# chao1224/GeoSSL

Hardware: AMD Instinct MI355X
Metric: molecules/s/GPU SchNet+DDM fwd+bwd (QM9-sized, bs=1024); % HBM roofline (higher is better)
Workload: dtype f32

## Files before the change

### geossl_amd/csrc/aggregate_reg.h

```cpp
#pragma once
#include "common.h"

namespace geossl {

typedef float f32x2 __attribute__((ext_vector_type(2)));

template <int NMAX, int RING_ = 0>
__device__ __forceinline__ void aggregate_reg_body(const float* __restrict__ x, const float* __restrict__ Wf,
                                                   const uint8_t* __restrict__ pair_flag, int a0, int n, int base,
                                                   int lane, int f, int F, int swap, float* __restrict__ out) {
#pragma clang fp contract(off)
  typedef f32x2 V;
#ifndef AGG_RING_SMALL
#define AGG_RING_SMALL 16
#endif
  constexpr int RING = RING_ > 0 ? RING_ : (NMAX > 26 ? 24 : (NMAX > 20 ? 20 : (NMAX > 18 ? 12 : AGG_RING_SMALL)));
  constexpr int NPOS = NMAX * (NMAX - 1) / 2;
  const float* __restrict__ wbase = Wf + (size_t)base * F;
  const bool has_cols = f >= 0;
  f = has_cols ? f : 0;
  if (n < 2) {
    if (n == 1 && has_cols) *reinterpret_cast<V*>(out + (size_t)a0 * F + f) = V(0.0f);
    return;
  }
  V xr[NMAX], acc[NMAX], ring[RING];
#pragma unroll
  for (int i = 0; i < NMAX; ++i) {
    xr[i] = *reinterpret_cast<const V*>(x + (size_t)(a0 + min(i, n - 1)) * F + f);
    acc[i] = V(0.0f);
  }
  const int nu = __builtin_amdgcn_readfirstlane(n);
  int rs_req = 0;
  auto load_row = [&](int a, int b) {
    asm volatile("" : "+s"(rs_req));
    const int slot = b < nu ? rs_req + (b - a - 1) : 0;
    const float* rowp = wbase + (size_t)slot * F;
    return __builtin_nontemporal_load(reinterpret_cast<const V*>(rowp + f));
  };
  auto next_pos = [&](int& a, int& b) {
    if (++b == NMAX) {
      rs_req += nu - a - 1;
      ++a;
      b = a + 1;
    }
  };
  unsigned flr[NMAX - 1];
#pragma unroll
  for (int a = 0; a < NMAX - 1; ++a) {
    const bool mine = lane > a && lane < n;
    flr[a] = pair_flag[base + (mine ? a * n - a * (a + 1) / 2 + lane - a - 1 : 0)];
  }
  int q = 0, ap = 0, bp = 1;
#pragma unroll
  for (int k = 0; k < RING && k < NPOS; ++k) {
    ring[k] = load_row(ap, bp);
    next_pos(ap, bp);
  }
#pragma unroll
  for (int a = 0; a < NMAX - 1; ++a) {
    const bool mine = lane > a && lane < n;
    unsigned fl = flr[a];
    asm volatile("" : "+v"(fl));
    fl = mine ? fl : 0u;
    if (swap) fl = ((fl & 1u) << 1) | ((fl >> 1) & 1u);
    const unsigned long long m0 = __builtin_amdgcn_ballot_w64((fl & 1u) != 0u);
    const unsigned long long m1 = __builtin_amdgcn_ballot_w64((fl & 2u) != 0u);
    V acc_a = acc[a];
    const V xa = xr[a];
#pragma unroll
    for (int b = a + 1; b < NMAX; ++b, ++q) {
      const V w = ring[q % RING];
      if (q + RING < NPOS) {
        ring[q % RING] = load_row(ap, bp);
        next_pos(ap, bp);
      }
      const V t0 = xr[b] * w;
      const V s0 = acc_a + t0;
      acc_a = ((m0 >> b) & 1ull) ? s0 : acc_a;
      const V t1 = xa * w;
      const V s1 = acc[b] + t1;
      acc[b] = ((m1 >> b) & 1ull) ? s1 : acc[b];
      asm volatile("" : "+v"(acc_a.x), "+v"(acc_a.y), "+v"(acc[b].x), "+v"(acc[b].y) : : "memory");
      __builtin_amdgcn_sched_barrier(0);
    }
    acc[a] = acc_a;
  }
#pragma unroll
  for (int i = 0; i < NMAX; ++i)
    if (i < n && has_cols) *reinterpret_cast<V*>(out + (size_t)(a0 + i) * F + f) = acc[i];
}

template <int NW = 4>
__device__ __forceinline__ void aggregate_block_body(const float* __restrict__ x, const float* __restrict__ Wf,
                                                     const uint8_t* __restrict__ pair_flag, int a0, int n, int base,
                                                     int swap, float* __restrict__ out, uint8_t* smem) {
#pragma clang fp contract(off)
  typedef f32x2 V;
  constexpr int F = 128, NP = 32;
  float* xs = reinterpret_cast<float*>(smem);
  uint8_t* fls = smem + 33 * F * sizeof(float);
  const int tid = threadIdx.x, lane = tid & 63;
  const int wave = __builtin_amdgcn_readfirstlane(tid >> 6);
  const int nu = __builtin_amdgcn_readfirstlane(n), np = nu * (nu - 1) / 2;
  for (int i = tid; i < nu * (F / 4); i += 64 * NW) {
    const int row = i >> 5, q = i & 31;
    *reinterpret_cast<f32x4*>(xs + row * F + 4 * q) = *reinterpret_cast<const f32x4*>(x + (size_t)(a0 + row) * F + 4 * q);
  }
  for (int p = tid; p < np; p += 64 * NW) {
    unsigned fl = pair_flag[base + p];
    if (swap) fl = ((fl & 1u) << 1) | ((fl >> 1) & 1u);
    fls[p] = (uint8_t)fl;
  }
  __syncthreads();
  if (nu < 2) {
    if (nu == 1 && wave == 0) *reinterpret_cast<V*>(out + (size_t)a0 * F + 2 * lane) = V(0.0f);
    return;
  }
  const float* __restrict__ wcol = Wf + (size_t)base * F + 2 * lane;
  const float* xl = xs + 2 * lane;
  int slot_l = 0, b_l = 0;
  unsigned long long mask = 0ull;
  auto describe = [&](int a) {
    const int u = lane < nu - 1 ? lane : 0;
    const int b = u + (u >= a ? 1 : 0);
    const int i = min(a, b), j = max(a, b);
    slot_l = nu > 1 ? i * nu - i * (i + 1) / 2 + (j - i - 1) : 0;
    b_l = nu > 1 ? b : 0;
    const unsigned fl = nu > 1 ? (unsigned)fls[slot_l] : 0u;
    const bool sends = lane < nu - 1 && ((a < b ? (fl & 1u) : (fl & 2u)) != 0u);
    mask = __builtin_amdgcn_ballot_w64(sends);
  };
  auto request = [&](V (&w)[NP]) {
#pragma unroll
    for (int u = 0; u < NP; ++u) {
      const int s = __builtin_amdgcn_readlane(slot_l, u);
      w[u] = __builtin_nontemporal_load(reinterpret_cast<const V*>(wcol + (size_t)s * F));
    }
  };
  auto reduce = [&](const V (&w)[NP], int a, unsigned long long m, int bl) {
    V acc = V(0.0f);
#pragma unroll
    for (int u = 0; u < NP; ++u) {
      const int b = __builtin_amdgcn_readlane(bl, u);
      const V xb = *reinterpret_cast<const V*>(xl + b * F);
      const V t = xb * w[u];
      const V s = acc + t;
      acc = ((m >> u) & 1ull) ? s : acc;
    }
    *reinterpret_cast<V*>(out + (size_t)(a0 + a) * F + 2 * lane) = acc;
  };
  V w0[NP], w1[NP];
  int a = wave;
  if (a < nu) {
    describe(a);
    request(w0);
  }
  while (a < nu) {
    const unsigned long long m0 = mask;
    const int bl0 = b_l;
    const int an = a + NW;
    if (an < nu) {
      describe(an);
      request(w1);
    }
    reduce(w0, a, m0, bl0);
    if (an >= nu) break;
    const unsigned long long m1 = mask;
    const int bl1 = b_l;
    const int an2 = an + NW;
    if (an2 < nu) {
      describe(an2);
      request(w0);
    }
    reduce(w1, an, m1, bl1);
    a = an2;
  }
}

__device__ __forceinline__ void aggregate_targets(const float* __restrict__ x, const float* __restrict__ Wf,
                                                  const uint8_t* __restrict__ pair_flag, int a0, int n, int base,
                                                  int lane, int f, int F, int swap, float* __restrict__ out, int t0,
                                                  int t1) {
#pragma clang fp contract(off)
  typedef f32x2 V;
  constexpr int NP = 32;
  const bool has_cols = f >= 0;
  f = has_cols ? f : 0;
  const int nu = __builtin_amdgcn_readfirstlane(n);
  if (nu < 2) {
    if (nu == 1 && t0 == 0 && t1 > 0 && has_cols) *reinterpret_cast<V*>(out + (size_t)a0 * F + f) = V(0.0f);
    return;
  }
  const float* __restrict__ wcol = Wf + (size_t)base * F + f;
  const float* __restrict__ xcol = x + (size_t)a0 * F + f;
  const uint8_t* __restrict__ flg = pair_flag + base;
  for (int a = t0; a < t1; ++a) {
    V acc = V(0.0f);
    for (int c0 = 0; c0 < nu - 1; c0 += NP) {
      const int u = min(c0 + (lane & (NP - 1)), nu - 2);
      const int b = u + (u >= a ? 1 : 0);
      const int i = min(a, b), j = max(a, b);
      const int slot = i * nu - i * (i + 1) / 2 + (j - i - 1);
      unsigned fl = flg[slot];
      if (swap) fl = ((fl & 1u) << 1) | ((fl >> 1) & 1u);
      const bool sends = lane < NP && c0 + lane < nu - 1 && ((a < b ? (fl & 1u) : (fl & 2u)) != 0u);
      const unsigned long long m = __builtin_amdgcn_ballot_w64(sends);
      V w[NP], xb[NP];
#pragma unroll
      for (int k = 0; k < NP; ++k) {
        const int sk = __builtin_amdgcn_readlane(slot, k), bk = __builtin_amdgcn_readlane(b, k);
        w[k] = *reinterpret_cast<const V*>(wcol + (size_t)sk * F);
        xb[k] = *reinterpret_cast<const V*>(xcol + (size_t)bk * F);
      }
      __builtin_amdgcn_sched_barrier(0);
#pragma unroll
      for (int k = 0; k < NP; ++k) {
        const V t = xb[k] * w[k];
        const V s2 = acc + t;
        acc = ((m >> k) & 1ull) ? s2 : acc;
      }
    }
    if (has_cols) *reinterpret_cast<V*>(out + (size_t)(a0 + a) * F + f) = acc;
  }
}

template <int NMAX, int K, int P>
__device__ __forceinline__ void aggregate_reg_part(const float* __restrict__ x, const float* __restrict__ Wf,
                                                   const uint8_t* __restrict__ pair_flag, int a0, int n, int base,
                                                   int lane, int f, int F, int swap, float* __restrict__ out) {
#pragma clang fp contract(off)
  typedef f32x2 V;
  constexpr int G0 = (P * NMAX) / K, G1 = ((P + 1) * NMAX) / K, NG = G1 - G0;
  constexpr int AEND = G1 < NMAX - 1 ? G1 : NMAX - 1;
  constexpr int RING = 40;
#define AGG_BS(a) ((a) < G0 ? G0 : (a) + 1)
#define AGG_BE(a) ((a) < G0 ? G1 : NMAX)
  constexpr int NPOS = G0 * NG + (AEND - G0) * NMAX - ((AEND * (AEND + 1)) / 2 - (G0 * (G0 + 1)) / 2);
  const bool has_cols = f >= 0;
  f = has_cols ? f : 0;
  const float* __restrict__ wbase = Wf + (size_t)base * F;
  V xr[NMAX], acc[NG], ring[RING];
#pragma unroll
// ... 96 lines not shown
```

### geossl_amd/csrc/chain.hip

```cpp
#include "common.h"
#include "geossl_hip.h"
#include "split.h"
#ifdef LOOP_TIMING
__device__ long long loop_dbg[2 * 1024];
__device__ int loop_dbg_n;
#define LOOP_MARK(tag)                                                                                     \
  do {                                                                                                     \
    if (blockIdx.x == 5 && threadIdx.x == 64) {                                                            \
      const int k_ = loop_dbg_n;                                                                           \
      if (k_ < 1024) {                                                                                     \
        loop_dbg[2 * k_] = (tag);                                                                          \
        loop_dbg[2 * k_ + 1] = (long long)__builtin_amdgcn_s_memrealtime();                                \
        loop_dbg_n = k_ + 1;                                                                               \
      }                                                                                                    \
    }                                                                                                      \
  } while (0)
#else
#define LOOP_MARK(tag) do {} while (0)
#endif
#include "aggregate_reg.h"

#include <cstdlib>

using namespace geossl;
// ... 342 lines not shown
#pragma unroll
      for (int s = 0; s < NS; ++s) {
        const GeosslChainStage st = ch.st[s];
        const uint32_t ro = rowc * (uint32_t)st.ld * 4u + 16u * kh;
#pragma unroll
        for (int mb = 0; mb < NMB; ++mb, ++cc) {
          f32x4 tp[4], rs[4];
          if (st.tprev != nullptr) {
            const char* tb = reinterpret_cast<const char*>(st.tprev) + 128 * mb;
#pragma unroll
            for (int q = 0; q < 4; ++q) tp[q] = *reinterpret_cast<const f32x4*>(tb + 32 * q + ro);
          }
          if (st.res != nullptr) {
            const char* rbp = reinterpret_cast<const char*>(st.res) + 128 * mb;
#pragma unroll
            for (int q = 0; q < 4; ++q) rs[q] = *reinterpret_cast<const f32x4*>(rbp + 32 * q + ro);
          }
          f32x16 acc;
#pragma unroll
          for (int q = 0; q < 4; ++q) {
            const f32x4 b = *reinterpret_cast<const f32x4*>(bias_s + s * F + 32 * mb + 8 * q + 4 * kh);
            acc[4 * q] = b.x; acc[4 * q + 1] = b.y; acc[4 * q + 2] = b.z; acc[4 * q + 3] = b.w;
          }
          {
            const u32x4* Ws = ring + (size_t)(cc % NSLOT) * CHUNK + lane;
            Frag3 af, an;
            af.h = Ws[0]; af.m = Ws[64]; af.l = Ws[128];
#pragma unroll
            for (int ks = 0; ks < KS; ++ks) {
              if (ks + 1 < KS) {
                const u32x4* src = Ws + (size_t)((ks + 1) * 3) * 64;
                an.h = src[0]; an.m = src[64]; an.l = src[128];
              }
              __builtin_amdgcn_sched_barrier(0);
              mma6(acc, af, xf[ks]);
              __builtin_amdgcn_sched_barrier(0);
              if (ks + 1 < KS) af = an;
            }
          }
          float v[16];
          epilogue(st, mb, acc, tp, rs, v);
          if (s + 1 < NS) {
            const float lo[8] = {v[0], v[1], v[2], v[3], v[4], v[5], v[6], v[7]};
            const float hi[8] = {v[8], v[9], v[10], v[11], v[12], v[13], v[14], v[15]};
            yf[2 * mb] = split8(lo);
            yf[2 * mb + 1] = split8(hi);
          }
          __syncthreads();
          store_v(st, mb, ro, live, v);
          if (cc + NSLOT < total) issue(cc + NSLOT);
        }
        if (s + 1 < NS) {
#pragma unroll
          for (int ks = 0; ks < KS; ++ks) xf[ks] = yf[ks];
        }
      }
    } else {
      const int m = wave - 4;
      const int rb = base + 4 * B + (int)blockIdx.x;
      const bool active = m < NMB && rb < nrb;
      const int row = 32 * rb + j;
      const bool live = active && row < R;
      const uint32_t rowc = (uint32_t)min(row, R - 1);
      if (active) {
        const char* xb = reinterpret_cast<const char*>(X) + 128 * m;
        const uint32_t xo = rowc * (uint32_t)ldx * 4u + 16u * kh;
        const f32x4 r0 = *reinterpret_cast<const f32x4*>(xb + xo), r1 = *reinterpret_cast<const f32x4*>(xb + 32 + xo);
        const f32x4 r2 = *reinterpret_cast<const f32x4*>(xb + 64 + xo), r3 = *reinterpret_cast<const f32x4*>(xb + 96 + xo);
        const float lo[8] = {r0.x, r0.y, r0.z, r0.w, r1.x, r1.y, r1.z, r1.w};
        const float hi[8] = {r2.x, r2.y, r2.z, r2.w, r3.x, r3.y, r3.z, r3.w};
        const Frag3 f0 = split8(lo), f1 = split8(hi);
        u32x4* xd = xchg + (size_t)CHUNK + (size_t)(2 * m * 3) * 64 + lane;
        xd[0] = f0.h; xd[64] = f0.m; xd[128] = f0.l;
        xd[192] = f1.h; xd[256] = f1.m; xd[320] = f1.l;
      }
      __syncthreads();
#pragma unroll
      for (int s = 0; s < NS; ++s) {
        const GeosslChainStage st = ch.st[s];
#pragma unroll
        for (int mbc = 0; mbc < NMB; ++mbc, ++cc) {
          float v[16];
          uint32_t ro = 0;
          if (active && mbc == 0) {
            const char* img = reinterpret_cast<const char*>(st.image) + (size_t)(m * KS) * 3 * 1024;
            const uint32_t voff = (uint32_t)lane * 16u;
            Frag3 af[KS];
#pragma unroll
            for (int ks = 0; ks < KS; ++ks) {
              const char* bk = img + ks * 3 * 1024;
              asm volatile("" : "+s"(bk));
              af[ks].h = *reinterpret_cast<const u32x4*>(bk + voff);
              af[ks].m = *reinterpret_cast<const u32x4*>(bk + 1024 + voff);
              af[ks].l = *reinterpret_cast<const u32x4*>(bk + 2048 + voff);
            }
            f32x4 tp[4], rs[4];
            ro = rowc * (uint32_t)st.ld * 4u + 16u * kh;
            if (st.tprev != nullptr) {
              const char* tb = reinterpret_cast<const char*>(st.tprev) + 128 * m;
#pragma unroll
              for (int q = 0; q < 4; ++q) tp[q] = *reinterpret_cast<const f32x4*>(tb + 32 * q + ro);
            }
            if (st.res != nullptr) {
              const char* rbp = reinterpret_cast<const char*>(st.res) + 128 * m;
#pragma unroll
              for (int q = 0; q < 4; ++q) rs[q] = *reinterpret_cast<const f32x4*>(rbp + 32 * q + ro);
            }
            f32x16 acc;
#pragma unroll
            for (int q = 0; q < 4; ++q) {
              const f32x4 b = *reinterpret_cast<const f32x4*>(bias_s + s * F + 32 * m + 8 * q + 4 * kh);
              acc[4 * q] = b.x; acc[4 * q + 1] = b.y; acc[4 * q + 2] = b.z; acc[4 * q + 3] = b.w;
            }
            {
              const u32x4* xs = xchg + (size_t)((s + 1) & 1) * CHUNK + lane;
              Frag3 xa, xn;
              xa.h = xs[0]; xa.m = xs[64]; xa.l = xs[128];
#pragma unroll
              for (int ks = 0; ks < KS; ++ks) {
                if (ks + 1 < KS) {
                  const u32x4* src = xs + (size_t)((ks + 1) * 3) * 64;
                  xn.h = src[0]; xn.m = src[64]; xn.l = src[128];
                }
                __builtin_amdgcn_sched_barrier(0);
                mma6(acc, af[ks], xa);
                __builtin_amdgcn_sched_barrier(0);
                if (ks + 1 < KS) xa = xn;
              }
            }
            epilogue(st, m, acc, tp, rs, v);
            if (s + 1 < NS) {
              const float lo[8] = {v[0], v[1], v[2], v[3], v[4], v[5], v[6], v[7]};
              const float hi[8] = {v[8], v[9], v[10], v[11], v[12], v[13], v[14], v[15]};
              const Frag3 f0 = split8(lo), f1 = split8(hi);
              u32x4* xd = xchg + (size_t)(s & 1) * CHUNK + (size_t)(2 * m * 3) * 64 + lane;
              xd[0] = f0.h; xd[64] = f0.m; xd[128] = f0.l;
              xd[192] = f1.h; xd[256] = f1.m; xd[320] = f1.l;
            }
          }
          __syncthreads();
          if (active && mbc == 0) store_v(st, m, ro, live, v);
          if (cc + NSLOT < total) issue(cc + NSLOT);
        }
      }
    }
  }
}

__device__ __forceinline__ float silu_f(float x) { return x / (1.0f + expf(-x)); }
__device__ __forceinline__ float dsilu_f(float x) {
  const float sg = 1.0f / (1.0f + expf(-x));
  return sg * (1.0f + x * (1.0f - sg));
}
template <int NS, int RB, int WPS, bool SILU, typename ChainT>
__device__ __forceinline__ void chain_cu_body(const ChainT& ch, const float* __restrict__ X, int ldx, int R,
                                              int row0, int row_end, int nloc) {
  constexpr int KS = 8, F = 128;
  constexpr int RBF = KS * 2 * 64;
#ifndef CHAIN_CU_NEB2
#define CHAIN_CU_NEB2 1
#endif
  constexpr int NEB = WPS == 1 ? 2 : CHAIN_CU_NEB2;
  extern __shared__ __attribute__((aligned(16))) uint8_t smem_raw[];
  u32x4* xbuf = reinterpret_cast<u32x4*>(smem_raw);
  float* bias_s = reinterpret_cast<float*>(xbuf + (size_t)RB * RBF);
  float* rmax = bias_s + NS * F;
  const int tid = threadIdx.x, lane = tid & 63, j = lane & 31, kh = lane >> 5;
  const int m = __builtin_amdgcn_readfirstlane(tid >> 6);
  const uint32_t voff = (uint32_t)lane * 16u;
  Frag2 af[KS];
  int eW = 0;
  float krow[RB];
  auto request_weights = [&](const auto& st) __attribute__((always_inline)) {
    const char* img = reinterpret_cast<const char*>(st.image) + (size_t)(m * KS) * 2 * 1024;
#pragma unroll
    for (int ks = 0; ks < KS; ++ks) {
      const char* bk = img + ks * 2 * 1024;
      asm volatile("" : "+s"(bk));
      af[ks].h = *reinterpret_cast<const u32x4*>(bk + voff);
      af[ks].l = *reinterpret_cast<const u32x4*>(bk + 1024 + voff);
    }
    eW = reinterpret_cast<const int*>(st.image)[4 * KS * 2 * 64 * 4 + m];
  };
  auto publish_max = [&](int i, float mx) __attribute__((always_inline)) {
    mx = fmaxf(mx, __shfl_xor(mx, 32, 64));
    if (kh == 0) rmax[(i * 4 + m) * 32 + j] = mx;
  };
  auto row_scale = [&](int i) __attribute__((always_inline)) {
    const float* r = rmax + (i * 4) * 32 + j;
    const float mx = fmaxf(fmaxf(r[0], r[32]), fmaxf(r[64], r[96]));
    const int e = mag_exponent(mx);
    krow[i] = __builtin_amdgcn_ldexpf(1.0f, e - 14);
    return __builtin_amdgcn_ldexpf(1.0f, 14 - e);
  };
  request_weights(ch.st[0]);
  for (int i = tid; i < NS * F; i += 256) {
    const int s = i / F;
    bias_s[i] = ch.st[s].bias != nullptr ? ch.st[s].bias[i - s * F] : 0.0f;
  }
  auto load_input = [&](const float* __restrict__ Xp, int ldxp) __attribute__((always_inline)) {
    f32x4 raw[RB][4];
    const char* xb = reinterpret_cast<const char*>(Xp) + 128 * m;
#pragma unroll
    for (int i = 0; i < RB; ++i) {
      const uint32_t rowc = (uint32_t)min(row0 + 32 * min(i, nloc - 1) + j, row_end - 1);
      const uint32_t xo = rowc * (uint32_t)ldxp * 4u + 16u * kh;
#pragma unroll
      for (int q = 0; q < 4; ++q) raw[i][q] = *reinterpret_cast<const f32x4*>(xb + 32 * q + xo);
    }
#pragma unroll
    for (int i = 0; i < RB; ++i) {
      if (i < nloc) {
        float mx = 0.0f;
#pragma unroll
        for (int q = 0; q < 4; ++q)
          mx = fmaxf(fmaxf(mx, fmaxf(fabsf(raw[i][q].x), fabsf(raw[i][q].y))), fmaxf(fabsf(raw[i][q].z), fabsf(raw[i][q].w)));
        publish_max(i, mx);
      }
    }
    lds_barrier();
#pragma unroll
    for (int i = 0; i < RB; ++i) {
      if (i < nloc) {
        const float sr = row_scale(i);
        const float lo[8] = {raw[i][0].x, raw[i][0].y, raw[i][0].z, raw[i][0].w,
                             raw[i][1].x, raw[i][1].y, raw[i][1].z, raw[i][1].w};
        const float hi[8] = {raw[i][2].x, raw[i][2].y, raw[i][2].z, raw[i][2].w,
                             raw[i][3].x, raw[i][3].y, raw[i][3].z, raw[i][3].w};
        const Frag2 f0 = split8h_scaled(lo, sr), f1 = split8h_scaled(hi, sr);
        u32x4* xd = xbuf + (size_t)i * RBF + (size_t)(2 * m * 2) * 64 + lane;
        xd[0] = f0.h; xd[64] = f0.l;
        xd[128] = f1.h; xd[192] = f1.l;
      }
    }
  };
  load_input(X, ldx);
  lds_barrier();
  LOOP_MARK(100);
  float vout[RB][16];
#pragma unroll
  for (int s = 0; s < NS; ++s) {
    const auto st = ch.st[s];
    const int eWs = eW;
    f32x4 tp[NEB][4], rs[NEB][4];
    const uint32_t nbytes = (uint32_t)R * (uint32_t)st.ld * 4u;
    const __amdgpu_buffer_rsrc_t rs_t = __builtin_amdgcn_make_buffer_rsrc(const_cast<float*>(st.tprev), 0, st.tprev != nullptr ? nbytes : 0u, 0x00020000);
    const __amdgpu_buffer_rsrc_t rs_r = __builtin_amdgcn_make_buffer_rsrc(const_cast<float*>(st.res), 0, st.res != nullptr ? nbytes : 0u, 0x00020000);
    const __amdgpu_buffer_rsrc_t rs_o = __builtin_amdgcn_make_buffer_rsrc(st.out, 0, st.out != nullptr ? nbytes : 0u, 0x00020000);
    const __amdgpu_buffer_rsrc_t rs_a = __builtin_amdgcn_make_buffer_rsrc(st.out_act, 0, (SILU && st.out_act != nullptr) ? nbytes : 0u, 0x00020000);
    const bool act_silu = SILU && (st.flags & GEOSSL_EPI_SILU) != 0;
    auto row_off = [&](int i) __attribute__((always_inline)) {
      const int row = row0 + 32 * i + j;
      return row < row_end ? (uint32_t)row * (uint32_t)st.ld * 4u + 128u * m + 16u * kh : 0xFFFFFF00u;
    };
    auto request_epi = [&](int i, f32x4 (&t)[4], f32x4 (&r)[4]) __attribute__((always_inline)) {
      const uint32_t ro = row_off(i);
#pragma unroll
      for (int q = 0; q < 4; ++q) t[q] = __builtin_bit_cast(f32x4, __builtin_amdgcn_raw_buffer_load_b128(rs_t, ro + 32 * q, 0, 0));
#pragma unroll
      for (int q = 0; q < 4; ++q) r[q] = __builtin_bit_cast(f32x4, __builtin_amdgcn_raw_buffer_load_b128(rs_r, ro + 32 * q, 0, 0));
    };
    auto store_rb = [&](int i) __attribute__((always_inline)) {
      const uint32_t ro = row_off(i);
#pragma unroll
      for (int q = 0; q < 4; ++q)
        __builtin_amdgcn_raw_buffer_store_b128(
            __builtin_bit_cast(u32x4, f32x4{vout[i][4 * q], vout[i][4 * q + 1], vout[i][4 * q + 2], vout[i][4 * q + 3]}), rs_o,
            ro + 32 * q, 0, 0);
      if constexpr (SILU) {
        float av[16];
#pragma unroll
        for (int e = 0; e < 16; ++e) av[e] = act_silu ? silu_f(vout[i][e]) : vout[i][e];
#pragma unroll
        for (int q = 0; q < 4; ++q)
          __builtin_amdgcn_raw_buffer_store_b128(
              __builtin_bit_cast(u32x4, f32x4{av[4 * q], av[4 * q + 1], av[4 * q + 2], av[4 * q + 3]}), rs_a, ro + 32 * q, 0, 0);
      }
    };
    if (NEB == 2) request_epi(0, tp[0], rs[0]);
#pragma unroll
    for (int i = 0; i < RB; ++i) {
      if (i < nloc) {
        if (NEB == 2) {
          if (i + 1 < nloc) request_epi(i + 1, tp[(i + 1) & 1], rs[(i + 1) & 1]);
        } else {
          request_epi(i, tp[0], rs[0]);
        }
        f32x16 acc;
#pragma unroll
        for (int e = 0; e < 16; ++e) acc[e] = 0.0f;
        {
          const u32x4* xs = xbuf + (size_t)i * RBF + lane;
          Frag2 xa, xn;
          xa.h = xs[0]; xa.l = xs[64];
#pragma unroll
          for (int ks = 0; ks < KS; ++ks) {
            if (ks + 1 < KS) {
              const u32x4* src = xs + (size_t)((ks + 1) * 2) * 64;
              xn.h = src[0]; xn.l = src[64];
            }
            __builtin_amdgcn_sched_barrier(0);
            acc = mfma_f16(af[ks].l, xa.h, acc);
            acc = mfma_f16(af[ks].h, xa.l, acc);
            acc = mfma_f16(af[ks].h, xa.h, acc);
            __builtin_amdgcn_sched_barrier(0);
            if (ks + 1 < KS) xa = xn;
          }
        }
        {
          const float kk = krow[i] * __builtin_amdgcn_ldexpf(1.0f, eWs - 14);
#pragma unroll
          for (int q = 0; q < 4; ++q) {
            const f32x4 bq = *reinterpret_cast<const f32x4*>(bias_s + s * F + 32 * m + 8 * q + 4 * kh);
            acc[4 * q] = fmaf(acc[4 * q], kk, bq.x);
            acc[4 * q + 1] = fmaf(acc[4 * q + 1], kk, bq.y);
            acc[4 * q + 2] = fmaf(acc[4 * q + 2], kk, bq.z);
            acc[4 * q + 3] = fmaf(acc[4 * q + 3], kk, bq.w);
          }
        }
        const f32x4(&t)[4] = tp[NEB == 2 ? (i & 1) : 0];
        const f32x4(&r)[4] = rs[NEB == 2 ? (i & 1) : 0];
        if (s > 0 && (st.flags & GEOSSL_CHAIN_ADD_PREV)) {
#pragma unroll
          for (int e = 0; e < 16; ++e) vout[i][e] += acc[e];
        } else {
#pragma unroll
          for (int e = 0; e < 16; ++e) vout[i][e] = acc[e];
        }
        if (st.flags & GEOSSL_EPI_SSP) {
#pragma unroll
          for (int e = 0; e < 16; ++e) vout[i][e] = ssp(vout[i][e]);
        }
        if (SILU && st.tprev != nullptr && (st.flags & GEOSSL_EPI_MUL_DSILU)) {
#pragma unroll
          for (int q = 0; q < 4; ++q) {
            vout[i][4 * q] *= dsilu_f(t[q].x);
            vout[i][4 * q + 1] *= dsilu_f(t[q].y);
            vout[i][4 * q + 2] *= dsilu_f(t[q].z);
            vout[i][4 * q + 3] *= dsilu_f(t[q].w);
          }
        } else if (st.tprev != nullptr) {
#pragma unroll
          for (int q = 0; q < 4; ++q) {
            vout[i][4 * q] *= dssp_from_out(t[q].x);
            vout[i][4 * q + 1] *= dssp_from_out(t[q].y);
            vout[i][4 * q + 2] *= dssp_from_out(t[q].z);
            vout[i][4 * q + 3] *= dssp_from_out(t[q].w);
          }
        }
        if (st.res != nullptr) {
#pragma unroll
          for (int q = 0; q < 4; ++q) {
            vout[i][4 * q] += r[q].x;
            vout[i][4 * q + 1] += r[q].y;
            vout[i][4 * q + 2] += r[q].z;
            vout[i][4 * q + 3] += r[q].w;
          }
        }
        if (s + 1 < NS) {
          float mx = 0.0f;
#pragma unroll
          for (int e = 0; e < 16; ++e) mx = fmaxf(mx, fabsf(vout[i][e]));
          publish_max(i, mx);
        }
        if (i > 0) store_rb(i - 1);
        if (i + 1 == nloc) store_rb(i);
      }
    }
    LOOP_MARK(110 + s);
    if (s + 1 < NS) {
      request_weights(ch.st[s + 1]);
      if (ch.st[s + 1].flags & GEOSSL_CHAIN_SAME_INPUT) continue;
      lds_barrier();
      if (ch.st[s + 1].flags & GEOSSL_CHAIN_NEW_INPUT) {
        load_input(ch.st[s + 1].xin, ch.st[s + 1].ldxin);
        lds_barrier();
        continue;
      }
#pragma unroll
      for (int i = 0; i < RB; ++i) {
        if (i < nloc) {
          const float sr = row_scale(i);
          float lo[8], hi[8];
#pragma unroll
          for (int e = 0; e < 8; ++e) {
            lo[e] = vout[i][e];
            hi[e] = vout[i][8 + e];
          }
          if constexpr (SILU) {
            if (st.flags & GEOSSL_EPI_SILU) {
#pragma unroll
              for (int e = 0; e < 8; ++e) {
                lo[e] = silu_f(lo[e]);
                hi[e] = silu_f(hi[e]);
              }
            }
          }
          const Frag2 f0 = split8h_scaled(lo, sr), f1 = split8h_scaled(hi, sr);
          u32x4* xd = xbuf + (size_t)i * RBF + (size_t)(2 * m * 2) * 64 + lane;
          xd[0] = f0.h; xd[64] = f0.l;
          xd[128] = f1.h; xd[192] = f1.l;
        }
      }
      lds_barrier();
    }
  }
}

template <int NS, int RB, int WPS, bool SILU>
__global__ __launch_bounds__(256, WPS) void k_row_chain_cu(GeosslChain ch, const float* __restrict__ X, int ldx, int R,
                                                           const int32_t* __restrict__ dyn_R) {
  R = dyn_count(R, dyn_R);
  const int nrb = (R + 31) / 32;
  const int nblk = (int)gridDim.x, base = nrb / nblk, extra = nrb - base * nblk, b = (int)blockIdx.x;
  const int rb0 = b * base + min(b, extra);
  const int nloc = base + (b < extra ? 1 : 0);
  if (nloc == 0) return;
  chain_cu_body<NS, RB, WPS, SILU>(ch, X, ldx, R, 32 * rb0, R, nloc);
}

struct LoopStage {
  const uint32_t* image;
  const float* bias;
  const float* res;
  const float* tprev;
  float* out;
  int flags, pad;
  static constexpr int ld = 128, ldxin = 0;
  static constexpr const float* xin = nullptr;
  static constexpr float* out_act = nullptr;
};
struct LoopOp {
  const float* X;
  const float* Wf;
  float* out;
  int kind, nstage, swap, pad;
  LoopStage st[3];
};
constexpr int LOOP_MAX_OPS = 14;
struct LoopArgs {
  LoopOp op[LOOP_MAX_OPS];
  const int4* plan;
  const int32_t* mol_ptr;
  const int32_t* pair_ptr;
  const uint8_t* pair_flag;
  int nops, R, stagger, pad;
  int nmol, mols_per_block;
};

template <int NMAX, int NW = 4>
__global__ __launch_bounds__(64 * NW, NW == 4 ? 2 : 1) void k_layer_loop(LoopArgs a) {
  constexpr int F = 128;
  int4 pl;
  if constexpr (NMAX > 0) {
    pl = a.plan[blockIdx.x];
  } else {
    pl.z = (int)blockIdx.x * a.mols_per_block;
    pl.w = min(pl.z + a.mols_per_block, a.nmol);
    if (pl.z >= pl.w) return;
    pl.x = a.mol_ptr[pl.z];
    pl.y = a.mol_ptr[pl.w];
    if (pl.x >= pl.y) return;
  }
  const int nloc = (pl.y - pl.x + 31) / 32;
  const int wave = __builtin_amdgcn_readfirstlane((int)threadIdx.x >> 6), lane = threadIdx.x & 63;
  if ((int)blockIdx.x >= ((int)gridDim.x + 1) / 2)
    for (int i = 0; i < a.stagger; ++i) __builtin_amdgcn_s_sleep(127);
  LOOP_MARK(1);
  for (int o = 0; o < a.nops; ++o) {
    const LoopOp& op = a.op[o];
    LOOP_MARK(10 + op.kind);
    if (op.kind == 0) {
      if (NW > 4 && wave >= 4) {
        for (int i = 0; i < 2 * op.nstage; ++i) __builtin_amdgcn_s_barrier();
      } else if (op.nstage == 1) chain_cu_body<1, 3, 2, false>(op, op.X, F, a.R, pl.x, pl.y, nloc);
      else if (op.nstage == 2) chain_cu_body<2, 3, 2, false>(op, op.X, F, a.R, pl.x, pl.y, nloc);
      else chain_cu_body<3, 3, 2, false>(op, op.X, F, a.R, pl.x, pl.y, nloc);
    } else {
      if constexpr (NMAX > 0 && NW == 4) {
        for (int mm = pl.z + wave; mm < pl.w; mm += 4) {
          const int a0 = a.mol_ptr[mm], n = a.mol_ptr[mm + 1] - a0, base = a.pair_ptr[mm];
          aggregate_reg_body<NMAX>(op.X, op.Wf, a.pair_flag, a0, n, base, lane, 2 * lane, F, op.swap, op.out);
        }
      } else {
        extern __shared__ __attribute__((aligned(16))) uint8_t loop_smem[];
        for (int mm = pl.z; mm < pl.w; ++mm) {
          const int a0 = a.mol_ptr[mm], n = a.mol_ptr[mm + 1] - a0, base = a.pair_ptr[mm];
          if (mm > pl.z) __syncthreads();
          aggregate_block_body<NW>(op.X, op.Wf, a.pair_flag, a0, n, base, op.swap, op.out, loop_smem);
        }
      }
    }
    LOOP_MARK(20);
    asm volatile("s_waitcnt vmcnt(0)" ::: "memory");
    LOOP_MARK(21);
    __syncthreads();
  }
  LOOP_MARK(2);
}

template <int KS>
int launch_chain(const GeosslChain& ch, const float* X, int ldx, int64_t R, hipStream_t stream,
                 const int32_t* dyn_R = nullptr) {
  constexpr int NMB = KS / 2, CHUNK_BYTES = KS * 3 * 1024;
  if (dyn_R != nullptr && KS != 8) return (int)hipErrorInvalidValue;
  const int nrb = (int)((R + 31) / 32), ngroups = (nrb + 3) / 4;
  const int nslot = chain_slots(ch.nstage * NMB);
  static const bool four_waves = getenv("GEOSSL_CHAIN4") != nullptr;
  static const bool eight_waves = getenv("GEOSSL_CHAIN8") != nullptr;
  const bool cu_form = KS == 8;
  const bool offsets32 = cu_form || !four_waves;
  bool same_input = false, silu = false;
  for (int s2 = 0; s2 < ch.nstage; ++s2) silu |= (ch.st[s2].flags & (GEOSSL_EPI_SILU | GEOSSL_EPI_MUL_DSILU)) != 0;
  if (ch.nstage > 3) silu = true;
  if (silu && !cu_form) return (int)hipErrorInvalidValue;
  for (int s2 = 0; s2 < ch.nstage; ++s2) {
    if (offsets32 && ((int64_t)R * ch.st[s2].ld * 4 >= (int64_t)0xFFFFFF00u || (int64_t)R * ldx * 4 >= (int64_t)0xFFFFFF00u ||
                      (int64_t)R * ch.st[s2].ldxin * 4 >= (int64_t)0xFFFFFF00u)) {
      if (dyn_R != nullptr) return (int)hipErrorInvalidValue;
      const int64_t r0 = ((R / 2 + 31) / 32) * 32;
      GeosslChain hi = ch;
      for (int s3 = 0; s3 < ch.nstage; ++s3) {
        GeosslChainStage& st = hi.st[s3];
        if (st.out != nullptr) st.out += r0 * st.ld;
        if (st.out_act != nullptr) st.out_act += r0 * st.ld;
        if (st.res != nullptr) st.res += r0 * st.ld;
        if (st.tprev != nullptr) st.tprev += r0 * st.ld;
        if (st.xin != nullptr) st.xin += r0 * st.ldxin;
      }
      const int rc = launch_chain<KS>(ch, X, ldx, r0, stream);
      return rc != 0 ? rc : launch_chain<KS>(hi, X + r0 * ldx, ldx, R - r0, stream);
    }
    same_input |= (ch.st[s2].flags & (GEOSSL_CHAIN_SAME_INPUT | GEOSSL_CHAIN_NEW_INPUT | GEOSSL_CHAIN_ADD_PREV)) != 0;
    if ((ch.st[s2].flags & GEOSSL_CHAIN_NEW_INPUT) && (ch.st[s2].xin == nullptr || ch.st[s2].ldxin < 16 * KS ||
                                                        (ch.st[s2].ldxin & 3)))
      return (int)hipErrorInvalidValue;
  }
  if (same_input && (!cu_form || (ch.st[0].flags & (GEOSSL_CHAIN_SAME_INPUT | GEOSSL_CHAIN_NEW_INPUT | GEOSSL_CHAIN_ADD_PREV))))
    return (int)hipErrorInvalidValue;
  if constexpr (KS == 8) {
    static const bool one_per_cu_env = getenv("GEOSSL_CHAIN_CU1") != nullptr;
    const bool one_per_cu = one_per_cu_env && !silu;
    static const int slots_env = getenv("GEOSSL_CHAIN_SLOTS") != nullptr ? atoi(getenv("GEOSSL_CHAIN_SLOTS")) : 0;
    const int RBV = one_per_cu ? 5 : 3, slots = slots_env > 0 ? slots_env : (one_per_cu ? 256 : 512);
    const int need = (nrb + RBV - 1) / RBV;
    const int fill = nrb < slots ? nrb : slots;
    const int grid = need > fill ? need : fill;
    const size_t lds = (size_t)RBV * KS * 2 * 1024 + (size_t)ch.nstage * 16 * KS * sizeof(float) + (size_t)RBV * 128 * sizeof(float);
#define LAUNCH_CU(NSV)                                                                                                 \
  do {                                                                                                                 \
    if (silu) {                                                                                                        \
      allow_big_lds(&k_row_chain_cu<NSV, 3, 2, true>);                                                                 \
      hipLaunchKernelGGL((k_row_chain_cu<NSV, 3, 2, true>), dim3(grid), dim3(256), lds, stream, ch, X, ldx, (int)R, dyn_R);   \
    } else if (one_per_cu) {                                                                                           \
      allow_big_lds(&k_row_chain_cu<NSV, 5, 1, false>);                                                                \
      hipLaunchKernelGGL((k_row_chain_cu<NSV, 5, 1, false>), dim3(grid), dim3(256), lds, stream, ch, X, ldx, (int)R, dyn_R);  \
    } else {                                                                                                           \
      allow_big_lds(&k_row_chain_cu<NSV, 3, 2, false>);                                                                \
      hipLaunchKernelGGL((k_row_chain_cu<NSV, 3, 2, false>), dim3(grid), dim3(256), lds, stream, ch, X, ldx, (int)R, dyn_R);  \
    }                                                                                                                  \
  } while (0)
#define LAUNCH_CU_LONG(NSV)                                                                                            \
  do {                                                                                                                 \
    allow_big_lds(&k_row_chain_cu<NSV, 3, 2, true>);                                                                   \
    hipLaunchKernelGGL((k_row_chain_cu<NSV, 3, 2, true>), dim3(grid), dim3(256), lds, stream, ch, X, ldx, (int)R, dyn_R);     \
  } while (0)
    switch (ch.nstage) {
      case 1: LAUNCH_CU(1); break;
      case 2: LAUNCH_CU(2); break;
      case 3: LAUNCH_CU(3); break;
      case 4: LAUNCH_CU_LONG(4); break;
      case 5: LAUNCH_CU_LONG(5); break;
      default: return (int)hipErrorInvalidValue;
    }
#undef LAUNCH_CU_LONG
#undef LAUNCH_CU
  } else if (four_waves) {
    const int grid = ngroups < 2048 ? ngroups : 2048;
    const size_t lds = (size_t)nslot * CHUNK_BYTES + (size_t)ch.nstage * 16 * KS * sizeof(float);
#define LAUNCH_NS(NSV)                                                                                           \
  do {                                                                                                           \
    allow_big_lds(&k_row_chain<KS, NSV>);                                                                        \
    hipLaunchKernelGGL((k_row_chain<KS, NSV>), dim3(grid), dim3(256), lds, stream, ch, X, ldx, (int)R);          \
  } while (0)
    switch (ch.nstage) {
      case 1: LAUNCH_NS(1); break;
      case 2: LAUNCH_NS(2); break;
      case 3: LAUNCH_NS(3); break;
      default: return (int)hipErrorInvalidValue;
    }
#undef LAUNCH_NS
  } else {
    const int want = (nrb + 4) / 5;
    const int grid = want < 256 ? want : 256;
    const size_t lds = (size_t)(nslot + 2) * CHUNK_BYTES + (size_t)ch.nstage * 16 * KS * sizeof(float);
#define LAUNCH_NS8(NSV)                                                                                          \
  do {                                                                                                           \
    allow_big_lds(&k_row_chain8<KS, NSV>);                                                                       \
    hipLaunchKernelGGL((k_row_chain8<KS, NSV>), dim3(grid), dim3(512), lds, stream, ch, X, ldx, (int)R);         \
  } while (0)
    switch (ch.nstage) {
      case 1: LAUNCH_NS8(1); break;
      case 2: LAUNCH_NS8(2); break;
      case 3: LAUNCH_NS8(3); break;
      default: return (int)hipErrorInvalidValue;
    }
#undef LAUNCH_NS8
  }
  GEOSSL_CHECK_LAUNCH();
  return 0;
}

}

#ifdef LOOP_TIMING
extern "C" int geossl_loop_debug_read(long long* host, int* n, int reset) {
  int rc = (int)hipMemcpyFromSymbol(host, HIP_SYMBOL(loop_dbg), sizeof(long long) * 2 * 1024);
  if (rc == 0) rc = (int)hipMemcpyFromSymbol(n, HIP_SYMBOL(loop_dbg_n), sizeof(int));
  if (rc == 0 && reset) {
    const int zero = 0;
    rc = (int)hipMemcpyToSymbol(HIP_SYMBOL(loop_dbg_n), &zero, sizeof(int));
  }
  return rc;
}
#endif
#ifdef CHAIN_TIMING
extern "C" int geossl_chain_debug_read(long long* host) {
  return (int)hipMemcpyFromSymbol(host, HIP_SYMBOL(chain_dbg), sizeof(long long) * 8 * 64);
}
#endif

extern "C" int64_t geossl_chain_image_words(int F) {
  if (F != 32 && F != 64 && F != 128) return 0;
  return (int64_t)(F / 32) * (F / 16) * 3 * 64 * 4;
}

extern "C" int geossl_chain_prepare(const GeosslPrepareBatch* batch, int nprob, int F, int transB, hipStream_t stream) {
  if (nprob <= 0) return 0;
  if (nprob > GEOSSL_PREPARE_MAX || geossl_chain_image_words(F) == 0) return (int)hipErrorInvalidValue;
  for (int z = 0; z < nprob; ++z)
    if (batch->ldw[z] != 0 && (batch->ldw[z] < F || (batch->ldw[z] & 3) || ((uintptr_t)batch->W[z] & 15)))
      return (int)hipErrorInvalidValue;
  const int KS = F / 16, nitems = (F / 32) * KS * 64;
  dim3 grid((nitems + 255) / 256, nprob);
  if (KS == 8) hipLaunchKernelGGL((k_chain_prepare<8>), grid, dim3(256), 0, stream, *batch, F, transB);
  else if (KS == 4) hipLaunchKernelGGL((k_chain_prepare<4>), grid, dim3(256), 0, stream, *batch, F, transB);
  else hipLaunchKernelGGL((k_chain_prepare<2>), grid, dim3(256), 0, stream, *batch, F, transB);
  GEOSSL_CHECK_LAUNCH();
  return 0;
}

extern "C" int geossl_linear_chain(const float* X, int ldx, const GeosslChain* chain, int64_t R, int F,
                                   hipStream_t stream) {
  return geossl_linear_chain_dyn(X, ldx, chain, R, F, nullptr, stream);
}

extern "C" int geossl_linear_chain_dyn(const float* X, int ldx, const GeosslChain* chain, int64_t R, int F,
                                       const int32_t* dyn_R, hipStream_t stream) {
  if (R <= 0) return 0;
  if (chain == nullptr || chain->nstage < 1 || chain->nstage > GEOSSL_CHAIN_MAX || geossl_chain_image_words(F) == 0)
    return (int)hipErrorInvalidValue;
  if (ldx < F || (ldx & 3)) return (int)hipErrorInvalidValue;
  for (int s = 0; s < chain->nstage; ++s) {
    const GeosslChainStage& st = chain->st[s];
    if (st.image == nullptr) return (int)hipErrorInvalidValue;
    if ((st.out != nullptr || st.res != nullptr || st.tprev != nullptr || st.out_act != nullptr) && (st.ld < F || (st.ld & 3)))
      return (int)hipErrorInvalidValue;
  }
  if (F == 128) return launch_chain<8>(*chain, X, ldx, R, stream, dyn_R);
  if (F == 64) return launch_chain<4>(*chain, X, ldx, R, stream, dyn_R);
  return launch_chain<2>(*chain, X, ldx, R, stream, dyn_R);
}

static int fill_loop_ops(const GeosslLoopOp* ops, int nops, int F, LoopArgs& a) {
  for (int o = 0; o < nops; ++o) {
    const GeosslLoopOp& src = ops[o];
    LoopOp& d = a.op[o];
    d.kind = src.kind; d.swap = src.swap; d.X = src.X; d.Wf = src.Wf; d.out = src.out; d.pad = 0;
    d.nstage = src.kind == 0 ? src.chain.nstage : 0;
    if (src.X == nullptr) return (int)hipErrorInvalidValue;
    if (src.kind == 0) {
      if (src.chain.nstage < 1 || src.chain.nstage > 3) return (int)hipErrorInvalidValue;
      for (int s2 = 0; s2 < 3; ++s2) {
        LoopStage& ls = d.st[s2];
        if (s2 < src.chain.nstage) {
          const GeosslChainStage& st = src.chain.st[s2];
          if (st.image == nullptr || (st.flags & ~(GEOSSL_EPI_BIAS | GEOSSL_EPI_SSP | GEOSSL_EPI_RESIDUAL | GEOSSL_EPI_MUL_DSSP)) ||
              ((st.out != nullptr || st.res != nullptr || st.tprev != nullptr) && st.ld != F) || st.xin != nullptr ||
              st.out_act != nullptr)
            return (int)hipErrorInvalidValue;
          ls.image = st.image; ls.bias = st.bias; ls.res = st.res; ls.tprev = st.tprev; ls.out = st.out; ls.flags = st.flags;
        } else {
          ls.image = nullptr; ls.bias = nullptr; ls.res = nullptr; ls.tprev = nullptr; ls.out = nullptr; ls.flags = 0;
        }
        ls.pad = 0;
      }
    } else if (src.kind == 1) {
      if (src.Wf == nullptr || src.out == nullptr) return (int)hipErrorInvalidValue;
      for (int s2 = 0; s2 < 3; ++s2) d.st[s2] = LoopStage{nullptr, nullptr, nullptr, nullptr, nullptr, 0, 0};
    } else {
      return (int)hipErrorInvalidValue;
    }
  }
  return 0;
}

static bool loop_wide(int64_t nblocks, bool one_molecule_per_block) {
  static int cus = 0;
  if (cus == 0) {
    int dev = 0, n = 0;
    cus = (hipGetDevice(&dev) == hipSuccess &&
           hipDeviceGetAttribute(&n, hipDeviceAttributeMultiprocessorCount, dev) == hipSuccess && n > 0) ? n : -1;
  }
  return one_molecule_per_block && cus > 0 && nblocks <= cus && getenv("GEOSSL_LOOP_NO_WIDE") == nullptr;
}

extern "C" int geossl_schnet_layer_loop(const GeosslLoopOp* ops, int nops, const int32_t* plan, int nblocks,
                                        const int32_t* mol_ptr, const int32_t* pair_ptr, const uint8_t* pair_flag,
                                        int max_n, int uniform, int64_t N, int F, int stagger, hipStream_t stream) {
  if (nops <= 0 || nblocks <= 0) return 0;
  if (ops == nullptr || plan == nullptr || nops > LOOP_MAX_OPS || F != 128 || !uniform || max_n > 20 || N <= 0)
    return (int)hipErrorInvalidValue;
  if (N * (int64_t)F * 4 >= (int64_t)0xFFFFFF00u) return (int)hipErrorInvalidValue;
  LoopArgs a;
  const int rc = fill_loop_ops(ops, nops, F, a);
  if (rc != 0) return rc;
  a.plan = reinterpret_cast<const int4*>(plan);
  a.mol_ptr = mol_ptr; a.pair_ptr = pair_ptr; a.pair_flag = pair_flag;
  a.nops = nops; a.R = (int)N; a.stagger = stagger; a.pad = 0; a.nmol = 0; a.mols_per_block = 0;
  const size_t lds = (size_t)3 * 8 * 2 * 1024 + (size_t)3 * 128 * sizeof(float) + (size_t)3 * 128 * sizeof(float);
  if (max_n <= 18) {
    allow_big_lds(&k_layer_loop<18>);
    hipLaunchKernelGGL((k_layer_loop<18>), dim3(nblocks), dim3(256), lds, stream, a);
  } else {
    allow_big_lds(&k_layer_loop<20>);
    hipLaunchKernelGGL((k_layer_loop<20>), dim3(nblocks), dim3(256), lds, stream, a);
  }
  GEOSSL_CHECK_LAUNCH();
  return 0;
}

extern "C" int geossl_schnet_layer_loop_ragged(const GeosslLoopOp* ops, int nops, const int32_t* mol_ptr,
                                               const int32_t* pair_ptr, const uint8_t* pair_flag, int64_t B,
                                               int mols_per_block, int64_t N, int F, hipStream_t stream) {
  if (nops <= 0 || B <= 0) return 0;
  if (ops == nullptr || mol_ptr == nullptr || pair_ptr == nullptr || nops > LOOP_MAX_OPS || F != 128 || N <= 0 ||
      mols_per_block < 1 || mols_per_block > 2)
    return (int)hipErrorInvalidValue;
  if (N * (int64_t)F * 4 >= (int64_t)0xFFFFFF00u) return (int)hipErrorInvalidValue;
  const int64_t nblocks = (B + mols_per_block - 1) / mols_per_block;
  if (nblocks > 1024) return (int)hipErrorInvalidValue;
  LoopArgs a;
  const int rc = fill_loop_ops(ops, nops, F, a);
  if (rc != 0) return rc;
  a.plan = nullptr;
  a.mol_ptr = mol_ptr; a.pair_ptr = pair_ptr; a.pair_flag = pair_flag;
  a.nops = nops; a.R = (int)N; a.stagger = 0; a.pad = 0; a.nmol = (int)B; a.mols_per_block = mols_per_block;
  const size_t lds = (size_t)3 * 8 * 2 * 1024 + (size_t)3 * 128 * sizeof(float) + (size_t)3 * 128 * sizeof(float);
  if (loop_wide(nblocks, mols_per_block == 1)) {
    allow_big_lds(&k_layer_loop<0, 8>);
    hipLaunchKernelGGL((k_layer_loop<0, 8>), dim3((unsigned)nblocks), dim3(512), lds, stream, a);
  } else {
    allow_big_lds(&k_layer_loop<0>);
    hipLaunchKernelGGL((k_layer_loop<0>), dim3((unsigned)nblocks), dim3(256), lds, stream, a);
  }
  GEOSSL_CHECK_LAUNCH();
  return 0;
}
```

Baseline: 411,900.

## Hand off intermediate activations between fused layer-loop ops through LDS

When one op in the persistent layer loop writes a buffer that the next op reads as input, the producer now also writes its output tile into shared memory using an XOR-swizzled row layout. The consumer (chain GEMM or pairwise aggregation) then reads it from LDS instead of global memory. This is meant to remove a global-memory round trip for intermediate activations within a block. Global writes are kept, and the change adds LDS stores plus extra barriers and relies on the LDS region not being overwritten between ops, which is a correctness risk.

```diff
diff --git a/geossl_amd/csrc/aggregate_reg.h b/geossl_amd/csrc/aggregate_reg.h
--- a/geossl_amd/csrc/aggregate_reg.h
+++ b/geossl_amd/csrc/aggregate_reg.h
@@ -5,12 +5,23 @@
 
 typedef float f32x2 __attribute__((ext_vector_type(2)));
 
-template <int NMAX, int RING_ = 0>
+__device__ __forceinline__ uint32_t raw_row_addr(uint32_t r, uint32_t p) { return r * 512u + (((p ^ r) & 31u) << 4); }
+
+template <int NMAX, int RING_ = 0, bool HANDOFF = false>
 __device__ __forceinline__ void aggregate_reg_body(const float* __restrict__ x, const float* __restrict__ Wf,
                                                    const uint8_t* __restrict__ pair_flag, int a0, int n, int base,
-                                                   int lane, int f, int F, int swap, float* __restrict__ out) {
+                                                   int lane, int f, int F, int swap, float* __restrict__ out,
+                                                   int lrow0 = 0, int hand = 0) {
 #pragma clang fp contract(off)
   typedef f32x2 V;
+  int hv = HANDOFF ? ((lrow0 << 2) | (hand & 3)) : 0;
+  if constexpr (HANDOFF) asm volatile("" : "+v"(hv));
+  const bool x_raw = HANDOFF && (hv & 1) != 0, out_raw = HANDOFF && (hv & 2) != 0;
+  lrow0 = hv >> 2;
+  auto raw_at = [&](int r) {
+    extern __shared__ __attribute__((aligned(16))) uint8_t agg_raw[];
+    return reinterpret_cast<V*>(agg_raw + raw_row_addr((uint32_t)r, (uint32_t)lane >> 1) + 8u * ((uint32_t)lane & 1u));
+  };
 #ifndef AGG_RING_SMALL
 #define AGG_RING_SMALL 16
 #endif
@@ -20,14 +31,25 @@
   const bool has_cols = f >= 0;
   f = has_cols ? f : 0;
   if (n < 2) {
-    if (n == 1 && has_cols) *reinterpret_cast<V*>(out + (size_t)a0 * F + f) = V(0.0f);
+    if (n == 1 && has_cols) {
+      *reinterpret_cast<V*>(out + (size_t)a0 * F + f) = V(0.0f);
+      if (out_raw) *raw_at(lrow0) = V(0.0f);
+    }
     return;
   }
   V xr[NMAX], acc[NMAX], ring[RING];
-#pragma unroll
-  for (int i = 0; i < NMAX; ++i) {
-    xr[i] = *reinterpret_cast<const V*>(x + (size_t)(a0 + min(i, n - 1)) * F + f);
-    acc[i] = V(0.0f);
+  if (x_raw) {
+#pragma unroll
+    for (int i = 0; i < NMAX; ++i) {
+      xr[i] = *raw_at(lrow0 + min(i, n - 1));
+      acc[i] = V(0.0f);
+    }
+  } else {
+#pragma unroll
+    for (int i = 0; i < NMAX; ++i) {
+      xr[i] = *reinterpret_cast<const V*>(x + (size_t)(a0 + min(i, n - 1)) * F + f);
+      acc[i] = V(0.0f);
+    }
   }
   const int nu = __builtin_amdgcn_readfirstlane(n);
   int rs_req = 0;
@@ -88,6 +110,11 @@
 #pragma unroll
   for (int i = 0; i < NMAX; ++i)
     if (i < n && has_cols) *reinterpret_cast<V*>(out + (size_t)(a0 + i) * F + f) = acc[i];
+  if (out_raw) {
+#pragma unroll
+    for (int i = 0; i < NMAX; ++i)
+      if (i < n) *raw_at(lrow0 + i) = acc[i];
+  }
 }
 
 template <int NW = 4>
diff --git a/geossl_amd/csrc/chain.hip b/geossl_amd/csrc/chain.hip
--- a/geossl_amd/csrc/chain.hip
+++ b/geossl_amd/csrc/chain.hip
@@ -518,9 +518,9 @@
   const float sg = 1.0f / (1.0f + expf(-x));
   return sg * (1.0f + x * (1.0f - sg));
 }
-template <int NS, int RB, int WPS, bool SILU, typename ChainT>
+template <int NS, int RB, int WPS, bool SILU, bool HAND = false, typename ChainT>
 __device__ __forceinline__ void chain_cu_body(const ChainT& ch, const float* __restrict__ X, int ldx, int R,
-                                              int row0, int row_end, int nloc) {
+                                              int row0, int row_end, int nloc, int hand = 0) {
   constexpr int KS = 8, F = 128;
   constexpr int RBF = KS * 2 * 64;
 #ifndef CHAIN_CU_NEB2
@@ -564,15 +564,25 @@
     const int s = i / F;
     bias_s[i] = ch.st[s].bias != nullptr ? ch.st[s].bias[i - s * F] : 0.0f;
   }
-  auto load_input = [&](const float* __restrict__ Xp, int ldxp) __attribute__((always_inline)) {
+  auto load_input = [&](const float* __restrict__ Xp, int ldxp, bool from_raw) __attribute__((always_inline)) {
     f32x4 raw[RB][4];
-    const char* xb = reinterpret_cast<const char*>(Xp) + 128 * m;
-#pragma unroll
-    for (int i = 0; i < RB; ++i) {
-      const uint32_t rowc = (uint32_t)min(row0 + 32 * min(i, nloc - 1) + j, row_end - 1);
-      const uint32_t xo = rowc * (uint32_t)ldxp * 4u + 16u * kh;
-#pragma unroll
-      for (int q = 0; q < 4; ++q) raw[i][q] = *reinterpret_cast<const f32x4*>(xb + 32 * q + xo);
+    if (HAND && from_raw) {
+#pragma unroll
+      for (int i = 0; i < RB; ++i) {
+        const uint32_t rl = (uint32_t)(min(row0 + 32 * min(i, nloc - 1) + j, row_end - 1) - row0);
+        const uint32_t ao = raw_row_addr(rl, (uint32_t)(8 * m + kh));
+#pragma unroll
+        for (int q = 0; q < 4; ++q) raw[i][q] = *reinterpret_cast<const f32x4*>(smem_raw + (ao ^ (32u * q)));
+      }
+    } else {
+      const char* xb = reinterpret_cast<const char*>(Xp) + 128 * m;
+#pragma unroll
+      for (int i = 0; i < RB; ++i) {
+        const uint32_t rowc = (uint32_t)min(row0 + 32 * min(i, nloc - 1) + j, row_end - 1);
+        const uint32_t xo = rowc * (uint32_t)ldxp * 4u + 16u * kh;
+#pragma unroll
+        for (int q = 0; q < 4; ++q) raw[i][q] = *reinterpret_cast<const f32x4*>(xb + 32 * q + xo);
+      }
     }
 #pragma unroll
     for (int i = 0; i < RB; ++i) {
@@ -600,7 +610,7 @@
       }
     }
   };
-  load_input(X, ldx);
+  load_input(X, ldx, (hand & 1) != 0);
   lds_barrier();
   LOOP_MARK(100);
   float vout[RB][16];
@@ -739,7 +749,7 @@
       if (ch.st[s + 1].flags & GEOSSL_CHAIN_SAME_INPUT) continue;
       lds_barrier();
       if (ch.st[s + 1].flags & GEOSSL_CHAIN_NEW_INPUT) {
-        load_input(ch.st[s + 1].xin, ch.st[s + 1].ldxin);
+        load_input(ch.st[s + 1].xin, ch.st[s + 1].ldxin, false);
         lds_barrier();
         continue;
       }
@@ -769,6 +779,21 @@
         }
       }
       lds_barrier();
+    }
+  }
+  if constexpr (HAND) {
+    if (hand & 2) {
+      lds_barrier();
+      const uint32_t ao = raw_row_addr((uint32_t)j, (uint32_t)(8 * m + kh));
+#pragma unroll
+      for (int i = 0; i < RB; ++i) {
+        if (i < nloc) {
+#pragma unroll
+          for (int q = 0; q < 4; ++q)
+            *reinterpret_cast<f32x4*>(smem_raw + (ao ^ (32u * q)) + 16384u * i) =
+                f32x4{vout[i][4 * q], vout[i][4 * q + 1], vout[i][4 * q + 2], vout[i][4 * q + 3]};
+        }
+      }
     }
   }
 }
@@ -817,6 +842,7 @@
 template <int NMAX, int NW = 4>
 __global__ __launch_bounds__(64 * NW, NW == 4 ? 2 : 1) void k_layer_loop(LoopArgs a) {
   constexpr int F = 128;
+  constexpr bool HAND = NMAX > 0 && NW == 4;
   int4 pl;
   if constexpr (NMAX > 0) {
     pl = a.plan[blockIdx.x];
@@ -839,14 +865,15 @@
     if (op.kind == 0) {
       if (NW > 4 && wave >= 4) {
         for (int i = 0; i < 2 * op.nstage; ++i) __builtin_amdgcn_s_barrier();
-      } else if (op.nstage == 1) chain_cu_body<1, 3, 2, false>(op, op.X, F, a.R, pl.x, pl.y, nloc);
-      else if (op.nstage == 2) chain_cu_body<2, 3, 2, false>(op, op.X, F, a.R, pl.x, pl.y, nloc);
-      else chain_cu_body<3, 3, 2, false>(op, op.X, F, a.R, pl.x, pl.y, nloc);
+      } else if (op.nstage == 1) chain_cu_body<1, 3, 2, false, HAND>(op, op.X, F, a.R, pl.x, pl.y, nloc, op.pad);
+      else if (op.nstage == 2) chain_cu_body<2, 3, 2, false, HAND>(op, op.X, F, a.R, pl.x, pl.y, nloc, op.pad);
+      else chain_cu_body<3, 3, 2, false, HAND>(op, op.X, F, a.R, pl.x, pl.y, nloc, op.pad);
     } else {
       if constexpr (NMAX > 0 && NW == 4) {
         for (int mm = pl.z + wave; mm < pl.w; mm += 4) {
           const int a0 = a.mol_ptr[mm], n = a.mol_ptr[mm + 1] - a0, base = a.pair_ptr[mm];
-          aggregate_reg_body<NMAX>(op.X, op.Wf, a.pair_flag, a0, n, base, lane, 2 * lane, F, op.swap, op.out);
+          aggregate_reg_body<NMAX, 0, true>(op.X, op.Wf, a.pair_flag, a0, n, base, lane, 2 * lane, F, op.swap, op.out,
+                                            a0 - pl.x, op.pad);
         }
       } else {
         extern __shared__ __attribute__((aligned(16))) uint8_t loop_smem[];
@@ -1068,6 +1095,16 @@
       return (int)hipErrorInvalidValue;
     }
   }
+  const char* env = getenv("GEOSSL_LOOP_HANDOFF");
+  const bool handoff = env == nullptr || atoi(env) != 0;
+  for (int o = 0; handoff && o + 1 < nops; ++o) {
+    const LoopOp& d = a.op[o];
+    const float* last = d.kind == 0 ? d.st[d.nstage - 1].out : d.out;
+    if (last != nullptr && a.op[o + 1].X == last) {
+      a.op[o].pad |= 2;
+      a.op[o + 1].pad |= 1;
+    }
+  }
   return 0;
 }
 
```

New measurement: 415,900 (median of 6 runs). Within noise of the previous version (+1.0%).
